# kdsuneraavinash/CH-Bin

Measured on AMD Instinct MI355X. Metric: convex-hull QP distances/sec (+ end-to-end bin-assign wall-clock), N=100000 D=136 B=64, higher is better.
Workload: dtype f64

## Files before the change

### ch-bin_amd/csrc/aux_kernels.hip

```cpp
#include "chb_internal.h"

namespace chb {
thread_local Gate g_gate;
namespace {

__global__ void fill_i32_kernel(int *p, int v, int n, Gate gate)
{
    CHB_GATE(gate);
    const int i = blockIdx.x * blockDim.x + threadIdx.x;
    if (i < n) p[i] = v;
}

__global__ void batch_close_kernel(int *labels, int *inb, const int *bq, const int *lab, int K)
{
    const int i = blockIdx.x * blockDim.x + threadIdx.x;
    if (i < K) {
        const int p = bq[i];
        labels[p] = lab[i];
        inb[p] = -1;
    }
}


__device__ __forceinline__ int member_key(int l, int p, const float4 *ms, const float *shell_inv, int nsh)
// ... 246 lines not shown
            const int e = atomicAdd(&cnt[rb[t]], 1);
            memb_id[e] = bq[i];
            memb_code[e] = -(i + 1);
        }
    }
    for (int i = tid + 1024 * kReg; i < K; i += 1024) {
        const int a = lab_prev[i];
        if (a >= 0 && a < B) {
            const int e = atomicAdd(&cnt[a], 1);
            memb_id[e] = bq[i];
            memb_code[e] = lab_old ? (i + 1) : (-(1 << 30) - i);
        }
        if (lab_old) {
            const int b = lab_old[i];
            if (b >= 0 && b < B) {
                const int e = atomicAdd(&cnt[b], 1);
                memb_id[e] = bq[i];
                memb_code[e] = -(i + 1);
            }
        }
    }
}

__global__ __launch_bounds__(256) void argmin_kernel(const double *dist, const int *lab_old, int *lab_prev,
                              int pos_begin, int pos_end, int B, int *lab_new, double *mind, double *second,
                              int *first_change, int in_place, Gate gate)
{
    CHB_GATE(gate);
    const int j = threadIdx.x & 7;
    const int pos = pos_begin + (int)((blockIdx.x * blockDim.x + threadIdx.x) >> 3);
    const bool valid = pos < pos_end;
    double best = kInf, runner = kInf;
    int bc = -1;
    if (valid) {
        const double *row = dist + (size_t)pos * B;
        for (int c = j; c < B; c += 8) {
            const double d = row[c];
            if (best > d) { runner = best; best = d; bc = c; }
            else if (runner > d) runner = d;
        }
    }
#pragma unroll
    for (int off = 1; off < 8; off <<= 1) {
        const double ob = __shfl_xor(best, off, 64), orr = __shfl_xor(runner, off, 64);
        const int oc = __shfl_xor(bc, off, 64);
        const bool take = ob < best || (ob == best && oc >= 0 && (bc < 0 || oc < bc));
// ... 363 lines not shown
}
void launch_batch_close(int *labels, int *inb, const int *bq, const int *lab, int K, hipStream_t s)
{
    if (K > 0) hipLaunchKernelGGL(batch_close_kernel, dim3((K + 255) / 256), dim3(256), 0, s, labels, inb, bq, lab, K);
}

void launch_bucket_base(const int *labels, int *inb, int N, int B, int *cnt, int *bin_ptr,
                        int *cursor, int *memb_id, int *pad_ptr, int *zero_me, hipStream_t s, const int *open_bq,
                        int open_K, int *open_lab_old, const SegPlan *seg, int *stats, const void *ms,
                        const float *shell_inv, int nsh)
{
    if (ms == nullptr || shell_inv == nullptr || nsh < 1) nsh = 1;
    const float4 *ms4 = reinterpret_cast<const float4 *>(ms);
    int blocks = (N + 255) / 256;
    if (blocks > 1024) blocks = 1024;
    hipLaunchKernelGGL(count_base_kernel, dim3(blocks), dim3(256), B * nsh * sizeof(int), s, labels, inb, N, B, cnt, open_bq,
                       open_K, open_lab_old, ms4, shell_inv, nsh, g_gate);
    hipLaunchKernelGGL(scan_kernel, dim3(1), dim3(256), 0, s, cnt, B, nsh, bin_ptr, cursor, pad_ptr, zero_me,
                       seg ? *seg : SegPlan{}, stats, g_gate);
    hipLaunchKernelGGL(fill_base_kernel, dim3((N + 255) / 256), dim3(256), 2 * B * nsh * sizeof(int), s, labels, inb, N, B,
                       cursor, memb_id, ms4, shell_inv, nsh, g_gate);
}

void launch_bucket_batch(const int *lab_prev, const int *lab_old, const int *bq, int K, int B,
                         int *cnt, int *bin_ptr, int *cursor, int *memb_id, int *memb_code, int *pad_ptr,
                         int *first_change, int *n_slow, int *nflag, hipStream_t s, void *bb_zero)
{
    (void)cnt; (void)cursor;
    hipLaunchKernelGGL(bucket_batch_kernel, dim3(1), dim3(1024), sizeof(int) * ((size_t)B + 2048), s, lab_prev,
                       lab_old, bq, K, B, bin_ptr, pad_ptr, memb_id, memb_code, first_change, n_slow, nflag,
                       reinterpret_cast<float4 *>(bb_zero), g_gate);
}

void launch_argmin(const double *dist, const int *lab_old, int *lab_prev, int pos_begin,
                   int pos_end, int B, int *lab_new, double *mind, double *second, int *first_change, bool in_place,
                   hipStream_t s)
{
    const int n = pos_end - pos_begin;
    if (n > 0)
        hipLaunchKernelGGL(argmin_kernel, dim3((n + 31) / 32), dim3(256), 0, s, dist, lab_old, lab_prev, pos_begin, pos_end, B,
                           lab_new, mind, second, first_change, in_place ? 1 : 0, g_gate);
}

}
```

### ch-bin_amd/csrc/chb_api.hip

```cpp
#include "chb_internal.h"
#include "../../include/chbin_hip.h"

#include <dlfcn.h>
#include <rccl/rccl.h>

#include <algorithm>
#include <cmath>
#include <cstdio>
#include <cstring>
#include <map>
#include <string>
#include <unordered_set>
#include <vector>

using namespace chb;

namespace {

thread_local std::string g_err;

int fail(int code, const std::string &msg)
{
    g_err = msg;
    return code;
// ... 92 lines not shown
    size_t cap = 0;
    hipError_t ensure(size_t n)
    {
        if (n <= cap) return hipSuccess;
        if (p) (void)hipHostFree(p);
        p = nullptr; cap = 0;
        hipError_t e = hipHostMalloc((void **)&p, std::max<size_t>(n, 1) * sizeof(T), hipHostMallocDefault);
        if (e == hipSuccess) cap = n;
        return e;
    }
    void release() { if (p) (void)hipHostFree(p); p = nullptr; cap = 0; }
    PinBuf() = default;
    PinBuf(const PinBuf &) = delete;
    PinBuf &operator=(const PinBuf &) = delete;
    ~PinBuf() { release(); }
};

}

struct PackBufs {
    DevBuf<unsigned short> Z;
    DevBuf<float> bias, sn, cs, cb, bb, tsn;
    DevBuf<int> pad_ptr;
    hipError_t ensure(size_t rows, size_t B, size_t Dz)
    {
        hipError_t e;
        if ((e = Z.ensure((rows + 64) * Dz)) != hipSuccess) return e;
        DevBuf<float> *f[] = {&bias, &sn, &cs, &cb};
        for (auto *b : f)
            if ((e = b->ensure(rows + 64)) != hipSuccess) return e;
        if ((e = bb.ensure(4 * B)) != hipSuccess) return e;
        if ((e = tsn.ensure(rows / 32 + B + 68)) != hipSuccess) return e;
        return pad_ptr.ensure(B + 1);
    }
    void release()
    {
        Z.release(); bias.release(); sn.release(); cs.release(); cb.release();
        bb.release(); tsn.release(); pad_ptr.release();
    }
    chb::MemberPack view()
    {
        return chb::MemberPack{Z.p, bias.p, sn.p, cs.p, cb.p, tsn.p, pad_ptr.p, reinterpret_cast<float4 *>(bb.p)};
    }
};

struct Switches {
    bool use_prefilter = true;
    bool allow_fused = true;
    bool fused_ptr64 = false;
    bool speculate = true;
    bool force_gather = false;
    bool allow_segments = true;
    bool fused_stripe = true;
    bool pp_allowed = true;
    bool pool_allowed = true, pool_force = false;
    bool allow_skip = true;
};

struct chb_ctx {
    int dev = 0;
    Switches sw;
// ... 99 lines not shown
    hipStream_t rc_copy = nullptr;
    hipEvent_t rc_up[2] = {nullptr, nullptr}, rc_done[2] = {nullptr, nullptr}, rc_down[2] = {nullptr, nullptr};
    DevBuf<int> xq, xhull, xcnt;
    DevBuf<double> xdist, xalpha, xpts;
    int prof = 0;
    std::map<std::string, ProfEntry> prof_acc;
    std::vector<Pending> pending;
    int64_t stats[4] = {0, 0, 0, 0};
    int64_t stats_seg_batches = 0;
    int64_t stats_lookahead = 0;
    int64_t stats_lookahead_failed = 0;
    ncclComm_t comm = nullptr;
    int rank = 0, world = 1;
    chb_allgather_fn hook = nullptr;
    void *hook_user = nullptr;
    std::vector<char> hook_send, hook_recv;
    double hint_base_members = 0.0, hint_batch_entries = 0.0;
#ifdef CHB_DEV_KNOBS
    struct DevKnobs {
        bool sl_bounds = false, sl_validate = false;
        int inject_short = 0, sl_bpw = 0, skip_never = 0;
        std::string sl_dbg;
        int64_t pack_rebuild_at = -1;
        bool hook_spec = false, local_verdict = false, skip_stats_on = false;
        int skip_stats[3] = {0, 0, 0};
        int batches = 0, launches = 0;
        DevBuf<int> viol, verr;
        DevBuf<unsigned long long> dbg;
    } dk;
#endif

    Lists L0() { return Lists{l0d.p, l0i.p, l0c.p}; }
    Lists L1() { return Lists{l1d.p, l1i.p, l1c.p}; }
    Lists L2() { return Lists{l2d.p, l2i.p, l2c.p}; }
    Lists Lcur() { return (round_in_batch & 1) ? L2() : L1(); }
    Lists Lprev() { return (round_in_batch & 1) ? L1() : L2(); }

    TopmArgs topm_args(int lo, int hi)
    {
        TopmArgs a{};
        a.X = X.p; a.Dp = Dp; a.bq = bq_cur; a.pos_begin = lo; a.pos_end = hi; a.B = B; a.m = m; a.Kcap = Kcap;
        return a;
    }
    ShortlistArgs shortlist_args(int lo, int hi)
    {
        ShortlistArgs a{};
// ... 111 lines not shown
    HIPCHK(h->bin_ptr.ensure(B + 1));
    HIPCHK(h->cursor.ensure(B * (size_t)kShells));
    HIPCHK(h->memb_id.ensure((size_t)h->N));
    HIPCHK(h->cnt2.ensure(B));
    HIPCHK(h->bin_ptr2.ensure(B + 1));
    HIPCHK(h->cursor2.ensure(B));
    HIPCHK(h->memb2_id.ensure(2 * K));
    HIPCHK(h->memb2_code.ensure(2 * K));
    if (h->pf_fit) {
        HIPCHK(h->cand.ensure(K * B * (size_t)kCandCap));
        HIPCHK(h->cand_cnt.ensure(K * B));
        HIPCHK(h->active.ensure(K * B));
        HIPCHK(h->n_active.ensure(1));
        HIPCHK(h->act_blk.ensure((K * B + 4095) / 4096 + 1));
        HIPCHK(h->flags64.ensure(B * ((K + kQTile - 1) / kQTile)));
        HIPCHK(h->flaglist.ensure(B * ((K + kQTile - 1) / kQTile)));
        HIPCHK(h->nflag.ensure(1));
        HIPCHK(h->flaglist2.ensure(B * ((K + kQTile - 1) / kQTile)));
        HIPCHK(h->nflag2.ensure(1));
        launch_fill_i32(h->flags64.p, 0, (int)(B * ((K + kQTile - 1) / kQTile)), h->stream);
        HIPCHK(h->overflow.ensure(1));
        HIPCHK(h->pk.ensure((size_t)h->N + 32 * B, B, (size_t)h->Dz));
        HIPCHK(h->pk2.ensure(2 * K + 32 * B, B, (size_t)h->Dz));
        h->seg_gcap = (int)std::min<size_t>(64, B / 4 + 1);
        HIPCHK(h->qord.ensure(K));
        HIPCHK(h->home.ensure(B));
        HIPCHK(h->seg_nseg.ensure(1));
        HIPCHK(h->seg_gflag.ensure(B));
        HIPCHK(h->seg_items.ensure(16 * (size_t)h->seg_gcap));
        if (h->fused) {
            for (int i = 0; i < 2; ++i) {
                HIPCHK(h->candu[i].ensure(K * B * (size_t)kCandCapU));
                HIPCHK(h->candu_cnt[i].ensure(K * B));
            }
            HIPCHK(h->slow.ensure(K * B));
            HIPCHK(h->n_slow.ensure(1));
            { const size_t had = h->short_cnt.cap; HIPCHK(h->short_cnt.ensure(1)); if (!had) HIPCHK(hipMemsetAsync(h->short_cnt.p, 0, sizeof(int), h->stream)); }
            HIPCHK(h->tau.ensure(K * B));
        }
    }
    h->Kcap = Kcap;
    return CHB_OK;
}

int fit_begin_impl(chb_ctx *h, int64_t B, const int64_t *initial, int m, bool sync = true)
{
// ... 138 lines not shown
void read_switches(chb_ctx *h)
{
    auto flag = [](const char *name, bool &v) { if (const char *e = getenv(name)) v = atoi(e) != 0; };
    Switches &w = h->sw;
    flag("CHB_PREFILTER", w.use_prefilter);
    flag("CHB_FUSED", w.allow_fused);
    flag("CHB_FUSED_PTR64", w.fused_ptr64);
    flag("CHB_SPECULATE", w.speculate);
    flag("CHB_FORCE_GATHER", w.force_gather);
    flag("CHB_SEGMENTS", w.allow_segments);
    flag("CHB_FUSED_STRIPE", w.fused_stripe);
    flag("CHB_PACK_INCR", w.pp_allowed);
    flag("CHB_TILE_SKIP", w.allow_skip);
    if (const char *e = getenv("CHB_POOL_TAU")) { w.pool_allowed = atoi(e) != 0; w.pool_force = atoi(e) == 2; }
#ifdef CHB_DEV_KNOBS
    auto &d = h->dk;
    d.sl_bounds = getenv("CHB_SL_BOUNDS") != nullptr;
    d.sl_validate = getenv("CHB_SL_VALIDATE") != nullptr;
    if (const char *e = getenv("CHB_SL_INJECT_SHORT")) d.inject_short = atoi(e);
    if (const char *e = getenv("CHB_SL_BPW")) d.sl_bpw = atoi(e);
    if (const char *e = getenv("CHB_SKIP_NEVER")) d.skip_never = atoi(e);
    if (const char *e = getenv("CHB_SL_DBG")) d.sl_dbg = e;
    if (const char *e = getenv("CHB_PACK_REBUILD_AT")) d.pack_rebuild_at = atoll(e);
    flag("CHB_DEV_HOOK_SPEC", d.hook_spec);
    flag("CHB_DEV_LOCAL_VERDICT", d.local_verdict);
    if (const char *e = getenv("CHB_DEV_SKIP_STATS"))
        d.skip_stats_on = sscanf(e, "%d,%d,%d", &d.skip_stats[0], &d.skip_stats[1], &d.skip_stats[2]) == 3;
#endif
}

#ifdef CHB_DEV_KNOBS
constexpr size_t kDbgWords = (size_t)65536 * 16;
int sl_bpw(const chb_ctx *h) { return h->dk.sl_bpw; }

int dev_shortlist_args(chb_ctx *h, ShortlistArgs &pa, bool skip_on, bool pp_now)
{
    auto &d = h->dk;
    if (skip_on && d.skip_never) pa.skip = 1 | 2 * d.skip_never;
    if (!d.sl_dbg.empty() && ++d.launches == 10) {
        HIPCHK(d.dbg.ensure(kDbgWords));
        HIPCHK(hipMemsetAsync(d.dbg.p, 0, kDbgWords * 8, h->stream));
        pa.dbg = d.dbg.p;
    }
    if (d.sl_bounds) {
        HIPCHK(d.viol.ensure(8));
        HIPCHK(hipMemsetAsync(d.viol.p, 0, 8 * sizeof(int), h->stream));
// ... 157 lines not shown
            RescoreArgs ra = h->rescore_args(q_lo, q_hi);
            ra.out = h->L0();
            Timed t(h, "rescore", (double)(q_hi - q_lo) * h->B);
            launch_rescore(ra, s);
        } else {
            a.out = Lists{nullptr, nullptr, nullptr};
            a.cand_out = h->cand.p; a.cand_cnt_out = h->cand_cnt.p; a.cand_cap = kCandCap;
            a.tau_out = h->tau.p; a.S = h->shadow_scale;
        }
        {
            Timed t(h, "topm_fallback", 0.0);
            launch_topm_flagged(a, h->flags64.p, fb_list, fb_n, s);
        }
        if (fusedp && !pp_now) { const int r_ = dev_shortlist_check(h, skip_on, qord_p); if (r_) return r_; }
    } else {
        Timed t(h, "topm_base", (double)(q_hi - q_lo) * h->hint_base_members);
        if (h->m > kMaxM) launch_topm_generic(a, s); else launch_topm(a, s);
    }
    HIPCHK(hipGetLastError());
    h->batch_open = true;
    return CHB_OK;
}

ShortlistArgs batch_entry_shortlist(chb_ctx *h, int lo, int hi)
{
    launch_pack_centered(h->X.p, h->D, h->Dp, h->memb2_id.p, h->memb2_code.p, h->bin_ptr2.p, h->B, 2 * h->K,
                         h->centers.p, h->mu_g.p, h->shadow_scale, h->Dz, h->pk2.view(), h->stream);
    ShortlistArgs pa = h->shortlist_args(lo, hi);
    pa.P = h->pk2.view(); pa.bin_ptr = h->bin_ptr2.p; pa.memb_id = h->memb2_id.p; pa.update = true;
    return pa;
}

void round_fused(chb_ctx *h, int lo, int hi, TopmArgs a)
{
    hipStream_t s = h->stream;
    const int cur = h->round_in_batch & 1;
    ShortlistArgs pa = batch_entry_shortlist(h, lo, hi);
    pa.tau_in = h->tau.p; pa.cand = h->candu[cur].p; pa.cand_cnt = h->candu_cnt[cur].p; pa.cand_cap = kCandCapU;
    {
        Timed t(h, "prefilter_update", (double)(hi - lo) * h->hint_batch_entries);
        launch_shortlist(pa, h->flags64.p, sl_bpw(h), s);
    }
    {
        a.in = a.out = Lists{nullptr, nullptr, nullptr};
        a.cand_out = h->candu[cur].p; a.cand_cnt_out = h->candu_cnt[cur].p; a.cand_cap = kCandCapU;
        Timed t(h, "topm_fallback", 0.0);
        launch_topm_flagged(a, h->flags64.p, h->flaglist.p, h->nflag.p, s);
    }
    FusedArgs f = h->fused_args(lo, hi);
    f.cand = h->cand.p; f.cand_cnt = h->cand_cnt.p; f.candu = h->candu[cur].p; f.candu_cnt = h->candu_cnt[cur].p;
    if (h->round_in_batch > 0) { f.candp = h->candu[cur ^ 1].p; f.candp_cnt = h->candu_cnt[cur ^ 1].p; }
    f.slow = h->slow.p; f.n_slow = h->n_slow.p; f.bin_ptr = h->bin_ptr.p; f.short_cnt = h->short_cnt.p;
// ... 38 lines not shown
        Timed t(h, "topm_fallback", 0.0);
        launch_topm_flagged(a, h->flags64.p, h->flaglist.p, h->nflag.p, s);
    }
    return CHB_OK;
}

void round_lists_plain(chb_ctx *h, int lo, int hi, const TopmArgs &a)
{
    Timed t(h, "topm_update", (double)(hi - lo) * h->hint_batch_entries);
    if (h->m > kMaxM) launch_topm_generic(a, h->stream); else launch_topm(a, h->stream);
}

int batch_round_dev(chb_ctx *h, int active)
{
    hipStream_t s = h->stream;
    const int lo = std::max(active, h->q_lo), hi = h->q_hi;
    if (hi <= lo) launch_fill_i32(h->fc_cur + kSlotFirstChange, h->K, 1, s);
    const bool fusedp = h->fused && h->lists_valid == false;
    if (hi > lo) {
        {
            Timed t(h, "bucket", (double)h->K);
            launch_bucket_batch(h->lab_prev.p, h->lab_old.p, h->bq_cur, h->K, h->B, h->cnt2.p, h->bin_ptr2.p, h->cursor2.p,
                                h->memb2_id.p, h->memb2_code.p, h->pk2.pad_ptr.p, h->fc_cur + kSlotFirstChange,
                                fusedp ? h->n_slow.p : nullptr, h->nflag.p, s, (h->pf_fit && h->pk2.bb.p) ? h->pk2.bb.p : nullptr);
        }
        TopmArgs a = h->topm_args(lo, hi);
        a.bin_ptr = h->bin_ptr2.p; a.memb_id = h->memb2_id.p; a.memb_code = h->memb2_code.p;
        a.in = h->L0(); a.out = h->Lcur();
        if (fusedp) round_fused(h, lo, hi, a);
        else {
            if (h->pf_fit && h->cand.p) { const int r_ = round_lists_shortlist(h, lo, hi, a); if (r_) return r_; }
            else round_lists_plain(h, lo, hi, a);
            QpArgs q = h->qp_args(lo, hi);
            q.lists = h->Lcur();
            q.prev = h->round_in_batch > 0 ? h->Lprev() : Lists{nullptr, nullptr, nullptr};
            Timed t(h, "hull_qp", (double)(hi - lo) * h->B);
            if (h->m > kMaxM) launch_hull_generic(q, s); else launch_hull_qp(q, s);
        }
        {
            Timed t(h, "argmin", (double)(hi - lo));
            launch_argmin(h->dist.p, h->lab_old.p, h->lab_prev.p, lo, hi, h->B, h->lab_new.p, h->mind.p,
                          h->want_margin ? h->mind2.p : nullptr, h->fc_cur + kSlotFirstChange, h->argmin_in_place, s);
        }
        h->stats[2] += (int64_t)(hi - lo) * h->B;
    }
    HIPCHK(hipGetLastError());
    h->stats[1] += 1;
// ... 1520 lines not shown
```

### ch-bin_amd/csrc/chb_internal.h

```cpp
#pragma once
#include <hip/hip_runtime.h>
#include <stdint.h>

#include <vector>

namespace chb {

struct Gate {
    const int *flag = nullptr;
    int need = 0;
};
extern thread_local Gate g_gate;
#define CHB_GATE(g) do { if ((g).flag != nullptr && *(g).flag < (g).need) return; } while (0)

constexpr double kInf = __builtin_huge_val();
constexpr int kMaxM = 16;
constexpr int kMaxMGeneric = 64;
constexpr int kQTile = 64;
constexpr int kPTile = 64;
constexpr int kKChunk = 8;
constexpr int kLdsStride = 66;

struct Lists {
    double *d;
// ... 11 lines not shown
    const int *bin_cnt = nullptr;
    const int *memb_code;
    int B, m, Kcap;
    Lists in;
    Lists out;
    int *cand_out = nullptr, *cand_cnt_out = nullptr;
    int cand_cap = 0;
    float *tau_out = nullptr;
    double S = 1.0;
};

void launch_topm(const TopmArgs &a, hipStream_t s);
void launch_topm_generic(const TopmArgs &a, hipStream_t s);
void launch_topm_flagged(const TopmArgs &a, int *flags64, const int *flaglist, const int *nflag, hipStream_t s);

constexpr int kCandCap = 128;
constexpr int kCandCapU = 32;

struct MemberPack {
    unsigned short *Z;
    float *bias;
    float *sn;
    float *cs, *cb;
    float *tsn;
    int *pad_ptr;
    float4 *bb;
    const int *nt = nullptr;
};
int shortlist_list_len(int m);
int shadow_row_elems(int D);
void launch_global_center(const double *X, int N, int D, int Dp, double *part, int part_blocks, double *mu_g,
                          unsigned int *rmax, hipStream_t s);
void launch_global_shadow(const double *X, int N, int D, int Dp, const double *mu_g, double S,
                          unsigned short *Gs, int Dz, void *gq, hipStream_t s);
void launch_bin_centers(const double *X, int D, int Dp, const int *memb_id, const int *bin_ptr, int B,
                        double *centers, hipStream_t s);
void launch_shell_scale(const void *ms, const int *memb_id, const int *bin_ptr, int B, int nsh, float *shell_inv,
                        hipStream_t s);
void launch_sample_shadow(const double *X, int D, int Dp, const int *ids, int n, int *labels,
                          int B, const double *centers, const double *mu_g, double S, unsigned short *Zs,
                          int Dz, void *ms, const int *new_lab, int *inb, hipStream_t s);
void launch_pack_centered(const double *X, int D, int Dp, const int *memb_id, const int *memb_code,
                          const int *bin_ptr, int B, int rows_hint, const double *centers, const double *mu_g,
                          double S, int Dz, const MemberPack &P, hipStream_t s);
void launch_pack_build(const unsigned short *Zs, const void *ms, int D, int Dz, const int *memb_id, const int *bin_ptr,
                       int B, int rows_hint, const MemberPack &P, bool shells, hipStream_t s);
void launch_query_norms(const double *X, int D, int Dp, int N, int B, const double *centers, double S, void *qn,
// ... 177 lines not shown
};
constexpr int kRecruitChunk = 16384;
constexpr int kRecruitMaxBins = 8192;
void launch_recruit(const RecruitArgs &a, hipStream_t s);
void launch_recruit_reduce(const double *dist, int nq, int B, int *bin, double *mind, double *margin, hipStream_t s);

void launch_fill_i32(int *p, int v, int n, hipStream_t s);
void launch_copy_i32(int *dst, const int *src, int n, hipStream_t s);
#ifdef CHB_DEV_KNOBS
void launch_validate_batch(const int *cand, const int *cand_cnt, int B, int Kcap, int pos_begin, int pos_end, int cap, int N,
                           const int *bin_ptr, const int *memb_id, const int *qord, int m, int *err, hipStream_t s);
void launch_inject_short(int *cand_cnt, int B, int Kcap, int pos, const int *bin_ptr, int m, hipStream_t s);
#endif
void launch_batch_close(int *labels, int *inb, const int *bq, const int *lab, int K, hipStream_t s);
void launch_bucket_base(const int *labels, int *inb, int N, int B, int *cnt, int *bin_ptr,
                        int *cursor, int *memb_id, int *pad_ptr, int *zero_me, hipStream_t s,
                        const int *open_bq = nullptr, int open_K = 0, int *open_lab_old = nullptr,
                        const SegPlan *seg = nullptr, int *stats = nullptr, const void *ms = nullptr,
                        const float *shell_inv = nullptr, int nsh = 1);
constexpr int kShells = 32;
constexpr int kMaxKeys = 8192;
void launch_bucket_batch(const int *lab_prev, const int *lab_old, const int *bq, int K, int B,
                         int *cnt, int *bin_ptr, int *cursor, int *memb_id, int *memb_code, int *pad_ptr,
                         int *first_change, int *n_slow, int *nflag, hipStream_t s, void *bb_zero = nullptr);
void launch_first_change(const int *lab_new, const int *lab_prev, int p0, int K, int *first_change,
                         hipStream_t s);
void launch_guess(const double *list_d, const int *list_cnt, const int *lab_old, int p0, int p1,
                  int B, int m, int Kcap, int *lab_prev, hipStream_t s);
void launch_guess_near(const float *tau, const int *lab_old, int p0, int p1, int B, int Kcap, int *lab_prev,
                       hipStream_t s);
enum SlotWord {
    kSlotFirstChange = 0,
    kSlotMaxTiles = 1,
    kSlotTotalTiles = 2,
    kSlotSkipped = 3,
    kSlotSeen = 4,
    kSlotUnloaded = 5,
    kSlotMark = 6,
    kSlotPoolCand = 7,
    kSlotPoolPairs = 8,
    kSlotHome = 9,
    kSlotShortCnt = 12,
    kSlotPackErr = 13,
};
constexpr int kSlotInts = 16;
enum FrameWord {
    kFrameTag = 0,
// ... 30 lines not shown
```

### ch-bin_amd/csrc/prefilter_kernels.hip

```cpp
#include "chb_internal.h"

#include <float.h>
#include <math.h>
#include <stdlib.h>

#include <algorithm>

namespace chb {
namespace {

using f16x8 = __attribute__((ext_vector_type(8))) _Float16;
using f32x16 = __attribute__((ext_vector_type(16))) float;
using f32x4 = __attribute__((ext_vector_type(4))) float;

constexpr int kBiasCols = 3;
constexpr int kBiasExp = 14;
constexpr float kGamma = 2.5e-5f;
constexpr float kSlack = 1e-6f;
constexpr int kPfW = 4;
constexpr int kPfQ = 32 * kPfW;
constexpr int kPfP = 32;
constexpr int kWideMaxSlices = 4;

__device__ __forceinline__ float round_up_f32(double v)
{
    float f = (float)v;
    if ((double)f < v) f = nextafterf(f, INFINITY);
    return f;
}

__device__ __forceinline__ unsigned short f16_shadow(double zs, double &back)
{
    float f = (float)zs;
    f = fminf(fmaxf(f, -65504.f), 65504.f);
    const _Float16 hv = (_Float16)f;
    back = (double)(float)hv;
    return __builtin_bit_cast(unsigned short, hv);
}

__device__ __forceinline__ void bound_max(float *slot, float v)
{
    if (v == v && v > 0.f) atomicMax(reinterpret_cast<unsigned int *>(slot), __float_as_uint(v));
}
// ... 975 lines not shown

template <int ML>
__device__ __forceinline__ void list_insert_desc(float (&l)[ML], float v)
{
#pragma unroll
    for (int i = 0; i < ML; ++i) {
        const float hi = fmaxf(l[i], v);
        v = fminf(l[i], v);
        l[i] = hi;
    }
}

__device__ __noinline__ void shortlist_flush_call(const unsigned *pool, int npark, int *cnt, const int *qpos, int *cand_bin,
                                                  int cand_cap, const int *memb, int lane)
{
    for (int i = lane; i < npark; i += 64) {
        const unsigned en = pool[i];
        const int qc = (int)(en >> 27), e = (int)(en & ((1u << 27) - 1u));
        const int off = atomicAdd(&cnt[qc], 1);
        if (off < cand_cap) cand_bin[(size_t)qpos[qc] * cand_cap + off] = memb[e];
    }
}

template <int ML, bool UPD, int KS, int SEG = 0, bool SKIP = false, bool POOL = false, bool WORK = false>
__global__ __launch_bounds__(64 * kPfW, (ML <= 5 && (KS == 9 || (!UPD && SEG != 2))) ? 4 : 3) void shortlist_kernel(ShortlistArgs a, int nqt, int nchunk,
                                                                         int bpw, int *flags64, int nqt64, Gate gate)
{
    CHB_GATE(gate);
    static_assert(!WORK || (!UPD && SEG == 0 && !SKIP && !POOL), "the work-list form is the plain base build");
    static_assert(SEG == 0 || !UPD, "segments exist for base members only");
    static_assert(!POOL || (!UPD && SEG == 0), "threshold pools serve the ordinary base launch");
#ifdef CHB_DEV_KNOBS
    const unsigned long long dbg_t0 = wall_clock64();
    int dbg_tiles = 0;
#endif
    constexpr int CPR = 2 * KS;
    constexpr int ROWB = 32 * KS;
    constexpr int TILEB = kPfP * ROWB;
    constexpr int METAB = 512;
    constexpr bool kFour = sl_four(KS, UPD, ML, SEG);
    constexpr int BUFB = kFour ? TILEB : TILEB + METAB;
    constexpr int NBUF = 3;
    constexpr int kPoolW = shortlist_pool_entries(ML);
    extern __shared__ __attribute__((aligned(16))) unsigned char smem[];
    unsigned *sPool = reinterpret_cast<unsigned *>(smem + NBUF * BUFB);
    int *sCnt = reinterpret_cast<int *>(sPool + kPfW * kPoolW);
// ... 93 lines not shown
        const int pch = (w + kPfW * j) * 64 + lane;
        const int r = pch / CPR, cs = pch - r * CPR;
        const int f = KS == 9 ? ((r >> 4) & 1) : ((r >> 2) & 3);
        src_off[j] = (r * CPR + (cs ^ f)) * 16;
    }
    int n_w = 0;
#pragma unroll
    for (int j = 0; j < 3; ++j) n_w += (w + kPfW * j < KS) ? 1 : 0;
    n_w += (UPD && w == 3) ? 1 : 0;
    n_w += (UPD && w == 2) ? 1 : 0;
    const unsigned char *zall = reinterpret_cast<const unsigned char *>(a.P.Z);

    int ic = c0, it = 0, isw = (UPD || SEG == 2) ? 1 : 0, ibuf = 0;
    int irow0 = 0, int_ = 0;
    bool ivalid = false;
    const long long pool_delta = (long long)reinterpret_cast<unsigned long long>(a.pool.Z) -
                                 (long long)reinterpret_cast<unsigned long long>(a.P.Z);
    long long ioff = 0;
    int brow0 = 0, bnt = 0;
#define CHB_SL_ISSUE_SEEK()                                                                        \
    {                                                                                              \
        ivalid = false;                                                                            \
        while (ic < c1) {                                                                          \
            irow0 = a.P.pad_ptr[ic];                                                               \
            int_ = a.P.nt != nullptr ? a.P.nt[ic] : (a.P.pad_ptr[ic + 1] - irow0) / kPfP;          \
            if (SEG == 0 && !UPD && a.seg.gflag != nullptr && a.seg.gflag[ic] >= 0) int_ = 0;     \
            if (SEG != 0) { irow0 += seg_tb * kPfP; int_ = min(int_, seg_te) - seg_tb; }           \
            if (int_ > 0) { ivalid = true; break; }                                                \
            ++ic;                                                                                  \
        }                                                                                          \
        if (POOL && ivalid) {                                                                      \
            brow0 = irow0; bnt = int_;                                                             \
            const bool pm_ = pool_mode_of(ic);                                                     \
            ioff = pm_ ? pool_delta + (long long)((ic * a.B + h_lo) * kPoolRows) * ROWB : (long long)irow0 * ROWB; \
            int_ = pm_ ? n_home : int_;                                                            \
        }                                                                                          \
    }
#ifdef CHB_DEV_KNOBS
#define CHB_SL_BOUNDS_DMA()                                                                        \
        if (a.viol != nullptr) {                                                                   \
            const long long bo_ = POOL ? ioff + (long long)it * kPfP * ROWB : (long long)row_ * ROWB; \
            const bool in_pack_ = bo_ >= 0 && bo_ + (long long)kPfP * ROWB <= a.viol_rows * ROWB;  \
            const bool in_pool_ = POOL && bo_ >= pool_delta && bo_ + (long long)kPfP * ROWB <= pool_delta + a.viol_pool_rows * ROWB; \
            if (!in_pack_ && !in_pool_) {                                                          \
                if (tid == 0 && atomicCAS(&a.viol[0], 0, 1) == 0) {                                \
                    a.viol[1] = ic; a.viol[2] = it; a.viol[3] = (int)(bo_ / ROWB); a.viol[4] = isw; a.viol[5] = int_; a.viol[6] = (int)(pool_delta >> 8); a.viol[7] = (int)blockIdx.x; \
                }                                                                                  \
                src_ = zall;                                                                       \
// ... 38 lines not shown
    int fbase0, fbase1;
    if (KS == 9) {
        const int f = (col >> 4) & 1;
        fbase0 = col * ROWB + ((h ^ f) << 4);
        fbase1 = fbase0 + 32;
    } else {
        const int f0 = (col >> 2) & 1, f1 = (col >> 3) & 1;
        fbase0 = col * ROWB + (f1 << 5) + ((h ^ f0) << 4);
        fbase1 = col * ROWB + ((1 ^ f1) << 5) + ((h ^ f0) << 4);
    }
    const unsigned ent0 = ((unsigned)col << 27) | (unsigned)(4 * h);

#ifdef CHB_DEV_KNOBS
#define CHB_SL_BOUNDS_FLUSH()                                                                      \
            if (a.viol != nullptr && ((long long)mb_ + e >= a.viol_members || e < 0)) {            \
                if (atomicCAS(&a.viol[0], 0, 2) == 0) { a.viol[1] = c; a.viol[2] = e; a.viol[3] = mb_; a.viol[4] = qc; a.viol[7] = (int)blockIdx.x; } \
                continue;                                                                          \
            }
#else
#define CHB_SL_BOUNDS_FLUSH()
#endif
#define CHB_SL_FLUSH()                                                                             \
    {                                                                                              \
        const int mb_ = a.bin_ptr[c];                                                              \
        const int npark_ = wcnt < kPoolW ? wcnt : kPoolW;                                          \
        if (SEG == 2) {                                                                            \
            for (int i = lane; i < npark_; i += 64)                                                \
                atomicAdd(&sCnt[32 * w + (int)(sPool[w * kPoolW + i] >> 27)], 1);                  \
            __builtin_amdgcn_fence(__ATOMIC_ACQ_REL, "wavefront");                                 \
            if (h == 0) {                                                                          \
                const int nq_ = sCnt[32 * w + col];                                                \
                int gb_ = 0;                                                                       \
                if (nq_ > 0 && qvalid) gb_ = atomicAdd(&a.cand_cnt[slot], nq_);                    \
                seg_over = seg_over || gb_ + nq_ > a.cand_cap;                                     \
                sGb[32 * w + col] = gb_;                                                           \
                sCnt[32 * w + col] = 0;                                                            \
            }                                                                                      \
            __builtin_amdgcn_fence(__ATOMIC_ACQ_REL, "wavefront");                                 \
        }                                                                                          \
        for (int i = lane; i < npark_; i += 64) {                                                  \
            const unsigned en = sPool[w * kPoolW + i];                                             \
            const int qc = (int)(en >> 27), e = (int)(en & ((1u << 27) - 1u));                     \
            int off = atomicAdd(&sCnt[32 * w + qc], 1);                                            \
            if (SEG == 2) off += sGb[32 * w + qc];                                                 \
            CHB_SL_BOUNDS_FLUSH()                                                                  \
            if (off < a.cand_cap)                                                                  \
                a.cand[(kSeated ? (size_t)c * a.Kcap + sQpos[32 * w + qc] : (size_t)c * a.Kcap + pos0 + 32 * w + qc) * a.cand_cap + off] = a.memb_id[mb_ + e]; \
        }                                                                                          \
        if (SEG == 2) {                                                                            \
            __builtin_amdgcn_fence(__ATOMIC_ACQ_REL, "wavefront");                                 \
            if (h == 0) sCnt[32 * w + col] = 0;                                                    \
        }                                                                                          \
    }
    int cbuf = 0;
    int wt_seen = 0, wt_skipped = 0, wt_unloaded = 0;
    int pool_cand = 0, pool_pairs = 0;
    for (int c = c0; c < c1; ++c) {
        const int row0 = a.P.pad_ptr[c];
        int ntile = a.P.nt != nullptr ? a.P.nt[c] : (a.P.pad_ptr[c + 1] - row0) / kPfP;
        if (SEG == 0 && !UPD && a.seg.gflag != nullptr && a.seg.gflag[c] >= 0) continue;
        if (SEG != 0) ntile = min(ntile, seg_te) - seg_tb;
        bool seg_over = false;
        const size_t slot = (size_t)c * a.Kcap + (qvalid ? qpos : a.pos_end - 1);
        float4 bb = a.P.bb[c];
        if (UPD) bb.y = sqrtf(bb.y) * (1.0f + 1e-6f);
        const float2 qn2 = a.qn[(size_t)sidx * a.B + c];
        const float E = ((UPD ? 1.2e-7f * bb.z : 2.0f * bb.w) + a.gamma * (1.001f * bb.z + 2.0f * snq * bb.y)) *
                        (1.0f + 4.0f * kSlack);
        const float rgq = rg * (1.0f + 4.0f * kSlack);
        const float *tsn_c = UPD ? nullptr : a.P.tsn + (row0 >> 5) + seg_tb;

        const float nj_hi = (qn2.x + E) * (1.0f + kSlack);
        const float nj_lo = (qn2.y - E) * (qn2.y > E ? (1.0f - kSlack) : (1.0f + kSlack));
        const float rsum = bb.x * (1.0f + kSlack);
        const float zn_lo = sqrtf(fmaxf(nj_lo, 0.f)) * (1.0f - 4.0f * kSlack) - rsum;
        float tau_run = INFINITY, hi_s1 = INFINITY;
#ifdef CHB_DEV_KNOBS
        const bool kSkipNever = (a.skip & 2) != 0;
        const bool kNoExit = (a.skip & 4) != 0, kNoWaveSkip = (a.skip & 8) != 0, kNoMidFlush = (a.skip & 16) != 0;
#else
        constexpr bool kSkipNever = false;
#endif
        constexpr bool can_skip = SKIP;
        float lb[ML];
// ... 380 lines not shown
#pragma unroll
    for (int j = 0; j < 3; ++j) {
        const int pch = (w + kPfW * j) * 64 + lane;
        const int r = pch / CPR, cs = pch - r * CPR;
        const int f = (r >> 4) & 1;
        src_off[j] = r * ROWB + (cs ^ f) * 16;
    }
    int n_w = 0;
#pragma unroll
    for (int j = 0; j < 3; ++j) n_w += (w + kPfW * j < KS) ? 1 : 0;
    n_w += (UPD && w == 3) ? 1 : 0;
    n_w += (UPD && w == 2) ? 1 : 0;
    const unsigned char *zall = reinterpret_cast<const unsigned char *>(a.P.Z);

    int ic = c0, it = 0, is = 0, isw = UPD ? 1 : 0, ibuf = 0;
    int irow0 = 0, int_ = 0;
    bool ivalid = false;
    int n_issued = 0, n_consumed = 0;
    auto issue_seek = [&]() __attribute__((always_inline)) {
        ivalid = false;
        while (ic < c1) {
            irow0 = a.P.pad_ptr[ic];
            int_ = a.P.nt != nullptr ? a.P.nt[ic] : (a.P.pad_ptr[ic + 1] - irow0) / kPfP;
            if (int_ > 0) { ivalid = true; break; }
            ++ic;
        }
    };
    auto issue = [&]() __attribute__((always_inline)) {
        unsigned char *dst_ = smem + ibuf * BUFB;
        const size_t row_ = (size_t)irow0 + (size_t)it * kPfP;
        const unsigned char *src_ = zall + row_ * ROWB + is * SLB;
#pragma unroll
        for (int j = 0; j < 3; ++j)
            if (w + kPfW * j < KS)
                __builtin_amdgcn_global_load_lds(src_ + src_off[j],
                    (__attribute__((address_space(3))) void *)(dst_ + (w + kPfW * j) * 1024), 16, 0, 0);
        if (UPD && w == 3) {
            const float *p_ = (h ? a.P.cs : a.P.bias) + row_ + col;
            __builtin_amdgcn_global_load_lds(p_, (__attribute__((address_space(3))) void *)(dst_ + TILEB), 4, 0, 0);
        }
        if (UPD && w == 2) {
            const float *p_ = (h ? a.P.sn : a.P.cb) + row_ + col;
            __builtin_amdgcn_global_load_lds(p_, (__attribute__((address_space(3))) void *)(dst_ + TILEB + 256), 4, 0, 0);
        }
        if (++ibuf == NBUF) ibuf = 0;
        ++n_issued;
        if (++is == NS) {
            is = 0;
            if (++it == int_) {
                it = 0;
                if (!UPD && isw == 0) isw = 1;
                else { isw = UPD ? 1 : 0; ++ic; issue_seek(); }
            }
        }
    };
    issue_seek();
    if (ivalid) issue();
    if (ivalid) issue();

    const int fbase0 = col * SLB + ((h ^ ((col >> 4) & 1)) << 4);
    const unsigned ent0 = ((unsigned)col << 27) | (unsigned)(4 * h);

    int cbuf = 0;
    for (int c = c0; c < c1; ++c) {
        const int row0 = a.P.pad_ptr[c];
        const int ntile = a.P.nt != nullptr ? a.P.nt[c] : (a.P.pad_ptr[c + 1] - row0) / kPfP;
        const size_t slot = (size_t)c * a.Kcap + (qvalid ? qpos : a.pos_end - 1);
        float4 bb = a.P.bb[c];
        if (UPD) bb.y = sqrtf(bb.y) * (1.0f + 1e-6f);
        const float2 qn2 = a.qn[(size_t)sidx * a.B + c];
        const float E = ((UPD ? 1.2e-7f * bb.z : 2.0f * bb.w) + a.gamma * (1.001f * bb.z + 2.0f * snq * bb.y)) *
                        (1.0f + 4.0f * kSlack);
        const float rgq = rg * (1.0f + 4.0f * kSlack);
        const float *tsn_c = UPD ? nullptr : a.P.tsn + (row0 >> 5);
        const float nj_hi = (qn2.x + E) * (1.0f + kSlack);
        const float nj_lo = (qn2.y - E) * (qn2.y > E ? (1.0f - kSlack) : (1.0f + kSlack));
        const float rsum = bb.x * (1.0f + kSlack);
        float lb[ML];
#pragma unroll
        for (int i = 0; i < ML; ++i) lb[i] = i < ML - m ? INFINITY : -INFINITY;
        float thr_s = -INFINITY;
        float thr2 = qvalid ? -FLT_MAX : INFINITY;
        if (UPD && qvalid) {
            float tau = INFINITY;
            if (a.tau_in != nullptr) tau = a.tau_in[slot];
            else if (a.seed.cnt[slot] >= m) tau = round_up_f32(a.seed.d[slot * m + m - 1] * a.S) * (1.0f + kSlack);
            if (tau < INFINITY) {
                const float hi = tau * (1.0f + 4.0f * kSlack) + rsum;
                thr2 = -0.5f * (hi * hi * (1.0f + 4.0f * kSlack) - nj_lo);
            }
        }
        if (h == 0) sCnt[32 * w + col] = 0;
        const bool tile_best = ntile >= a.tile_best_min && 4 * ntile >= m * m && !(!UPD && a.skip != 0);
        const int kmax = (ML > 8 && !tile_best && ntile >= a.tile_best_min && !(!UPD && a.skip != 0)) ? a.tile_k2 : 0x7fffffff;
        int wcnt = 0;
        auto flush = [&]() __attribute__((always_inline)) {
            const int mb_ = a.bin_ptr[c];
            const int npark_ = wcnt < kPoolW ? wcnt : kPoolW;
            for (int i = lane; i < npark_; i += 64) {
                const unsigned en = sPool[w * kPoolW + i];
                const int qc = (int)(en >> 27), e = (int)(en & ((1u << 27) - 1u));
                const int off = atomicAdd(&sCnt[32 * w + qc], 1);
                if (off < a.cand_cap)
                    a.cand[((size_t)c * a.Kcap + pos0 + 32 * w + qc) * a.cand_cap + off] = a.memb_id[mb_ + e];
            }
        };

        for (int sweep = UPD ? 1 : 0; sweep < 2; ++sweep) {
            const float rgs = (sweep ? rg : -rg) * (1.0f + kSlack);
            if (!UPD && sweep == 1) {
                float mg[ML];
#pragma unroll
                for (int i = 0; i < ML; ++i) mg[i] = lb[i];
#pragma unroll
                for (int i = 0; i < ML; ++i) {
                    const float o = __shfl_xor(lb[i], 32, 64);
                    list_insert_desc<ML>(mg, i >= ML - m ? o : -INFINITY);
                }
                const float ms = mg[ML - 1];
                float tau = INFINITY;
// ... 437 lines not shown
```

Measured before the change: 647.4 million.

## Order batch-entry buckets by query position and restrict shortlist scans to per-tile windows

```diff
diff --git a/ch-bin_amd/csrc/aux_kernels.hip b/ch-bin_amd/csrc/aux_kernels.hip
--- a/ch-bin_amd/csrc/aux_kernels.hip
+++ b/ch-bin_amd/csrc/aux_kernels.hip
@@ -292,6 +292,141 @@
     }
 }
 
+__device__ __forceinline__ int scan_parts_wave(int *part, int lane)
+{
+    int loc = 0;
+    for (int i = 0; i < 16; ++i) loc += part[16 * lane + i];
+    int inc = loc;
+#pragma unroll
+    for (int off = 1; off < 64; off <<= 1) {
+        const int o = __shfl_up(inc, off, 64);
+        if (lane >= off) inc += o;
+    }
+    int run = inc - loc;
+    for (int i = 0; i < 16; ++i) {
+        const int v = part[16 * lane + i];
+        part[16 * lane + i] = run;
+        run += v;
+    }
+    return run;
+}
+
+__global__ __launch_bounds__(1024) void bucket_batch_ordered_kernel(const int *lab_prev, const int *lab_old, const int *bq,
+                                                                    int K, int B, int nch, int shift, int q_lo,
+                                                                    int q_hi, int *bin_ptr, int *pad_ptr, int *memb_id,
+                                                                    int *memb_code, int4 *twin,
+                                                                    int *first_change, int *n_slow, int *nflag,
+                                                                    float4 *bb_zero, Gate gate)
+{
+    CHB_GATE(gate);
+    extern __shared__ int sh[];
+    const int ncell = 2 * B * nch;
+    int *cnt = sh, *part = sh + ncell + 1;
+    const int tid = threadIdx.x;
+    if (bb_zero != nullptr)
+        for (int b = tid; b < B; b += 1024) bb_zero[b] = make_float4(0.f, 0.f, 0.f, 0.f);
+    if (tid == 0) {
+        if (first_change) *first_change = K;
+        if (n_slow) *n_slow = 0;
+        if (nflag) *nflag = 0;
+    }
+    for (int c = tid; c < ncell; c += 1024) cnt[c] = 0;
+    __syncthreads();
+    auto cell_of = [&](int l, int run, int i) { return (l >= 0 && l < B) ? (2 * l + run) * nch + (i >> shift) : -1; };
+    constexpr int kReg = 8;
+    int ra[kReg], rb[kReg];
+#pragma unroll
+    for (int t = 0; t < kReg; ++t) {
+        const int i = tid + 1024 * t;
+        ra[t] = i < K ? cell_of(lab_prev[i], 1, i) : -1;
+        rb[t] = i < K ? cell_of(lab_old[i], 0, i) : -1;
+    }
+#pragma unroll
+    for (int t = 0; t < kReg; ++t) {
+        if (ra[t] >= 0) atomicAdd(&cnt[ra[t]], 1);
+        if (rb[t] >= 0) atomicAdd(&cnt[rb[t]], 1);
+    }
+    for (int i = tid + 1024 * kReg; i < K; i += 1024) {
+        const int a = cell_of(lab_prev[i], 1, i), b = cell_of(lab_old[i], 0, i);
+        if (a >= 0) atomicAdd(&cnt[a], 1);
+        if (b >= 0) atomicAdd(&cnt[b], 1);
+    }
+    __syncthreads();
+    {
+        const int per = (ncell + 1023) / 1024;
+        const int c0 = min(ncell, tid * per), c1 = min(ncell, c0 + per);
+        int s = 0;
+        for (int c = c0; c < c1; ++c) s += cnt[c];
+        part[tid] = s;
+        __syncthreads();
+        if (tid < 64) {
+            const int total = scan_parts_wave(part, tid);
+            if (tid == 63) { cnt[ncell] = total; bin_ptr[B] = total; }
+        }
+        __syncthreads();
+        int run = part[tid];
+        for (int c = c0; c < c1; ++c) { const int v = cnt[c]; cnt[c] = run; run += v; }
+        __syncthreads();
+    }
+    {
+        const int per = (B + 1023) / 1024;
+        const int b0 = min(B, tid * per), b1 = min(B, b0 + per);
+        int sp = 0;
+        for (int b = b0; b < b1; ++b) sp += (cnt[(2 * b + 2) * nch] - cnt[2 * b * nch] + 31) / 32 * 32;
+        part[tid] = sp;
+        __syncthreads();
+        if (tid < 64) {
+            const int ptotal = scan_parts_wave(part, tid);
+            if (tid == 63) pad_ptr[B] = ptotal;
+        }
+        __syncthreads();
+        int prun = part[tid];
+        for (int b = b0; b < b1; ++b) {
+            bin_ptr[b] = cnt[2 * b * nch];
+            pad_ptr[b] = prun;
+            prun += (cnt[(2 * b + 2) * nch] - cnt[2 * b * nch] + 31) / 32 * 32;
+        }
+    }
+    __syncthreads();
+    const int nqt = (q_hi - q_lo + kSlQTile - 1) / kSlQTile;
+    for (int x = tid; x < B * nqt; x += 1024) {
+        const int b = x / nqt, t = x - b * nqt;
+        const int p0 = q_lo + t * kSlQTile, p1 = min(p0 + kSlQTile, q_hi) - 1;
+        const int e0 = cnt[2 * b * nch];
+        const int tb = (cnt[2 * b * nch + (p0 >> shift)] - e0) >> 5;
+        const int te = (cnt[(2 * b + 1) * nch + (p1 >> shift) + 1] - e0 + 31) >> 5;
+        twin[x] = make_int4(pad_ptr[b] + 32 * tb, te - tb, e0 + 32 * tb, 0);
+    }
+    __syncthreads();
+#pragma unroll
+    for (int t = 0; t < kReg; ++t) {
+        const int i = tid + 1024 * t;
+        if (ra[t] >= 0) {
+            const int e = atomicAdd(&cnt[ra[t]], 1);
+            memb_id[e] = bq[i];
+            memb_code[e] = i + 1;
+        }
+        if (rb[t] >= 0) {
+            const int e = atomicAdd(&cnt[rb[t]], 1);
+            memb_id[e] = bq[i];
+            memb_code[e] = -(i + 1);
+        }
+    }
+    for (int i = tid + 1024 * kReg; i < K; i += 1024) {
+        const int a = cell_of(lab_prev[i], 1, i), b = cell_of(lab_old[i], 0, i);
+        if (a >= 0) {
+            const int e = atomicAdd(&cnt[a], 1);
+            memb_id[e] = bq[i];
+            memb_code[e] = i + 1;
+        }
+        if (b >= 0) {
+            const int e = atomicAdd(&cnt[b], 1);
+            memb_id[e] = bq[i];
+            memb_code[e] = -(i + 1);
+        }
+    }
+}
+
 __global__ __launch_bounds__(256) void argmin_kernel(const double *dist, const int *lab_old, int *lab_prev,
                               int pos_begin, int pos_end, int B, int *lab_new, double *mind, double *second,
                               int *first_change, int in_place, Gate gate)
@@ -701,11 +836,31 @@
                        cursor, memb_id, ms4, shell_inv, nsh, g_gate);
 }
 
+int batch_window_shift(int K, int B, int cells)
+{
+    if (K <= 0 || B <= 0) return 0;
+    for (int shift = 7; shift < 31; ++shift) {
+        const long long nch = ((K - 1) >> shift) + 1;
+        if (2LL * B * nch <= cells) return shift;
+        if (nch == 1) break;
+    }
+    return 0;
+}
+
 void launch_bucket_batch(const int *lab_prev, const int *lab_old, const int *bq, int K, int B,
                          int *cnt, int *bin_ptr, int *cursor, int *memb_id, int *memb_code, int *pad_ptr,
-                         int *first_change, int *n_slow, int *nflag, hipStream_t s, void *bb_zero)
+                         int *first_change, int *n_slow, int *nflag, hipStream_t s, void *bb_zero, int *twin, int twin_shift,
+                         int q_lo, int q_hi)
 {
     (void)cnt; (void)cursor;
+    if (twin != nullptr && K > 0 && q_lo >= 0 && q_lo < q_hi && q_hi <= K) {
+        const int nch = ((K - 1) >> twin_shift) + 1;
+        hipLaunchKernelGGL(bucket_batch_ordered_kernel, dim3(1), dim3(1024), sizeof(int) * (2 * (size_t)B * nch + 1 + 1024), s,
+                           lab_prev, lab_old, bq, K, B, nch, twin_shift, q_lo, q_hi, bin_ptr, pad_ptr, memb_id, memb_code,
+                           reinterpret_cast<int4 *>(twin), first_change, n_slow, nflag, reinterpret_cast<float4 *>(bb_zero),
+                           g_gate);
+        return;
+    }
     hipLaunchKernelGGL(bucket_batch_kernel, dim3(1), dim3(1024), sizeof(int) * ((size_t)B + 2048), s, lab_prev,
                        lab_old, bq, K, B, bin_ptr, pad_ptr, memb_id, memb_code, first_change, n_slow, nflag,
                        reinterpret_cast<float4 *>(bb_zero), g_gate);
diff --git a/ch-bin_amd/csrc/chb_api.hip b/ch-bin_amd/csrc/chb_api.hip
--- a/ch-bin_amd/csrc/chb_api.hip
+++ b/ch-bin_amd/csrc/chb_api.hip
@@ -138,6 +138,8 @@
     DevBuf<unsigned short> Z;
     DevBuf<float> bias, sn, cs, cb, bb, tsn;
     DevBuf<int> pad_ptr;
+    DevBuf<int> twin;
+    hipError_t ensure_windows(size_t B, size_t K) { return twin.ensure(4 * B * ((K + kSlQTile - 1) / kSlQTile + 1)); }
     hipError_t ensure(size_t rows, size_t B, size_t Dz)
     {
         hipError_t e;
@@ -152,7 +154,7 @@
     void release()
     {
         Z.release(); bias.release(); sn.release(); cs.release(); cb.release();
-        bb.release(); tsn.release(); pad_ptr.release();
+        bb.release(); tsn.release(); pad_ptr.release(); twin.release();
     }
     chb::MemberPack view()
     {
@@ -298,6 +300,7 @@
         int inject_short = 0, sl_bpw = 0, skip_never = 0;
         std::string sl_dbg;
         int64_t pack_rebuild_at = -1;
+        int batch_cells = -1;
         bool hook_spec = false, local_verdict = false, skip_stats_on = false;
         int skip_stats[3] = {0, 0, 0};
         int batches = 0, launches = 0;
@@ -455,6 +458,7 @@
         HIPCHK(h->overflow.ensure(1));
         HIPCHK(h->pk.ensure((size_t)h->N + 32 * B, B, (size_t)h->Dz));
         HIPCHK(h->pk2.ensure(2 * K + 32 * B, B, (size_t)h->Dz));
+        HIPCHK(h->pk2.ensure_windows(B, K));
         h->seg_gcap = (int)std::min<size_t>(64, B / 4 + 1);
         HIPCHK(h->qord.ensure(K));
         HIPCHK(h->home.ensure(B));
@@ -639,6 +643,7 @@
     if (const char *e = getenv("CHB_SKIP_NEVER")) d.skip_never = atoi(e);
     if (const char *e = getenv("CHB_SL_DBG")) d.sl_dbg = e;
     if (const char *e = getenv("CHB_PACK_REBUILD_AT")) d.pack_rebuild_at = atoll(e);
+    if (const char *e = getenv("CHB_BATCH_CELLS")) d.batch_cells = std::max(0, std::min(atoi(e), kBatchCells));
     flag("CHB_DEV_HOOK_SPEC", d.hook_spec);
     flag("CHB_DEV_LOCAL_VERDICT", d.local_verdict);
     if (const char *e = getenv("CHB_DEV_SKIP_STATS"))
@@ -842,12 +847,22 @@
     return CHB_OK;
 }
 
+int entry_window_shift(const chb_ctx *h, int lo, int hi)
+{
+    if (!h->pf_fit || h->pk2.twin.p == nullptr || lo < 0 || lo >= hi || hi > h->K) return 0;
+#ifdef CHB_DEV_KNOBS
+    if (h->dk.batch_cells >= 0) return batch_window_shift(h->K, h->B, h->dk.batch_cells);
+#endif
+    return batch_window_shift(h->K, h->B);
+}
+
 ShortlistArgs batch_entry_shortlist(chb_ctx *h, int lo, int hi)
 {
     launch_pack_centered(h->X.p, h->D, h->Dp, h->memb2_id.p, h->memb2_code.p, h->bin_ptr2.p, h->B, 2 * h->K,
                          h->centers.p, h->mu_g.p, h->shadow_scale, h->Dz, h->pk2.view(), h->stream);
     ShortlistArgs pa = h->shortlist_args(lo, hi);
     pa.P = h->pk2.view(); pa.bin_ptr = h->bin_ptr2.p; pa.memb_id = h->memb2_id.p; pa.update = true;
+    pa.P.twin = entry_window_shift(h, lo, hi) ? reinterpret_cast<const int4 *>(h->pk2.twin.p) : nullptr;
     return pa;
 }
 
@@ -932,7 +947,8 @@
             Timed t(h, "bucket", (double)h->K);
             launch_bucket_batch(h->lab_prev.p, h->lab_old.p, h->bq_cur, h->K, h->B, h->cnt2.p, h->bin_ptr2.p, h->cursor2.p,
                                 h->memb2_id.p, h->memb2_code.p, h->pk2.pad_ptr.p, h->fc_cur + kSlotFirstChange,
-                                fusedp ? h->n_slow.p : nullptr, h->nflag.p, s, (h->pf_fit && h->pk2.bb.p) ? h->pk2.bb.p : nullptr);
+                                fusedp ? h->n_slow.p : nullptr, h->nflag.p, s, (h->pf_fit && h->pk2.bb.p) ? h->pk2.bb.p : nullptr,
+                                entry_window_shift(h, lo, hi) ? h->pk2.twin.p : nullptr, entry_window_shift(h, lo, hi), lo, hi);
         }
         TopmArgs a = h->topm_args(lo, hi);
         a.bin_ptr = h->bin_ptr2.p; a.memb_id = h->memb2_id.p; a.memb_code = h->memb2_code.p;
diff --git a/ch-bin_amd/csrc/chb_internal.h b/ch-bin_amd/csrc/chb_internal.h
--- a/ch-bin_amd/csrc/chb_internal.h
+++ b/ch-bin_amd/csrc/chb_internal.h
@@ -57,7 +57,10 @@
     float *bias;
     float *sn;
     float *cs, *cb;
-    float *tsn;
+    union {
+        float *tsn;
+        const int4 *twin;
+    };
     int *pad_ptr;
     float4 *bb;
     const int *nt = nullptr;
@@ -281,7 +284,11 @@
 constexpr int kMaxKeys = 8192;
 void launch_bucket_batch(const int *lab_prev, const int *lab_old, const int *bq, int K, int B,
                          int *cnt, int *bin_ptr, int *cursor, int *memb_id, int *memb_code, int *pad_ptr,
-                         int *first_change, int *n_slow, int *nflag, hipStream_t s, void *bb_zero = nullptr);
+                         int *first_change, int *n_slow, int *nflag, hipStream_t s, void *bb_zero = nullptr,
+                         int *twin = nullptr, int twin_shift = 0, int q_lo = 0, int q_hi = 0);
+constexpr int kSlQTile = 128;
+constexpr int kBatchCells = 14336;
+int batch_window_shift(int K, int B, int cells = kBatchCells);
 void launch_first_change(const int *lab_new, const int *lab_prev, int p0, int K, int *first_change,
                          hipStream_t s);
 void launch_guess(const double *list_d, const int *list_cnt, const int *lab_old, int p0, int p1,
diff --git a/ch-bin_amd/csrc/prefilter_kernels.hip b/ch-bin_amd/csrc/prefilter_kernels.hip
--- a/ch-bin_amd/csrc/prefilter_kernels.hip
+++ b/ch-bin_amd/csrc/prefilter_kernels.hip
@@ -19,6 +19,7 @@
 constexpr float kSlack = 1e-6f;
 constexpr int kPfW = 4;
 constexpr int kPfQ = 32 * kPfW;
+static_assert(kPfQ == kSlQTile, "the batch-entry tile windows are per query tile of the shortlist kernels");
 constexpr int kPfP = 32;
 constexpr int kWideMaxSlices = 4;
 
@@ -1040,6 +1041,8 @@
     }
 }
 
+__device__ __forceinline__ int4 entry_window(const MemberPack &P, int c, int nqt, int qt) { return P.twin[c * nqt + qt]; }
+
 template <int ML, bool UPD, int KS, int SEG = 0, bool SKIP = false, bool POOL = false, bool WORK = false>
 __global__ __launch_bounds__(64 * kPfW, (ML <= 5 && (KS == 9 || (!UPD && SEG != 2))) ? 4 : 3) void shortlist_kernel(ShortlistArgs a, int nqt, int nchunk,
                                                                          int bpw, int *flags64, int nqt64, Gate gate)
@@ -1179,8 +1182,13 @@
     {                                                                                              \
         ivalid = false;                                                                            \
         while (ic < c1) {                                                                          \
+            if (UPD && a.P.twin != nullptr) {                                                      \
+                const int4 win_ = entry_window(a.P, ic, nqt, qt);                                  \
+                irow0 = win_.x; int_ = win_.y;                                                     \
+            } else {                                                                               \
             irow0 = a.P.pad_ptr[ic];                                                               \
             int_ = a.P.nt != nullptr ? a.P.nt[ic] : (a.P.pad_ptr[ic + 1] - irow0) / kPfP;          \
+            }                                                                                      \
             if (SEG == 0 && !UPD && a.seg.gflag != nullptr && a.seg.gflag[ic] >= 0) int_ = 0;     \
             if (SEG != 0) { irow0 += seg_tb * kPfP; int_ = min(int_, seg_te) - seg_tb; }           \
             if (int_ > 0) { ivalid = true; break; }                                                \
@@ -1265,7 +1273,7 @@
 #endif
 #define CHB_SL_FLUSH()                                                                             \
     {                                                                                              \
-        const int mb_ = a.bin_ptr[c];                                                              \
+        const int mb_ = (UPD && a.P.twin != nullptr) ? entry_window(a.P, c, nqt, qt).z : a.bin_ptr[c]; \
         const int npark_ = wcnt < kPoolW ? wcnt : kPoolW;                                          \
         if (SEG == 2) {                                                                            \
             for (int i = lane; i < npark_; i += 64)                                                \
@@ -1303,6 +1311,7 @@
         int ntile = a.P.nt != nullptr ? a.P.nt[c] : (a.P.pad_ptr[c + 1] - row0) / kPfP;
         if (SEG == 0 && !UPD && a.seg.gflag != nullptr && a.seg.gflag[c] >= 0) continue;
         if (SEG != 0) ntile = min(ntile, seg_te) - seg_tb;
+        if (UPD && a.P.twin != nullptr) ntile = entry_window(a.P, c, nqt, qt).y;
         bool seg_over = false;
         const size_t slot = (size_t)c * a.Kcap + (qvalid ? qpos : a.pos_end - 1);
         float4 bb = a.P.bb[c];
@@ -1729,6 +1738,10 @@
         while (ic < c1) {
             irow0 = a.P.pad_ptr[ic];
             int_ = a.P.nt != nullptr ? a.P.nt[ic] : (a.P.pad_ptr[ic + 1] - irow0) / kPfP;
+            if (UPD && a.P.twin != nullptr) {
+                const int4 win = entry_window(a.P, ic, nqt, qt);
+                irow0 = win.x; int_ = win.y;
+            }
             if (int_ > 0) { ivalid = true; break; }
             ++ic;
         }
@@ -1771,7 +1784,8 @@
     int cbuf = 0;
     for (int c = c0; c < c1; ++c) {
         const int row0 = a.P.pad_ptr[c];
-        const int ntile = a.P.nt != nullptr ? a.P.nt[c] : (a.P.pad_ptr[c + 1] - row0) / kPfP;
+        int ntile = a.P.nt != nullptr ? a.P.nt[c] : (a.P.pad_ptr[c + 1] - row0) / kPfP;
+        if (UPD && a.P.twin != nullptr) ntile = entry_window(a.P, c, nqt, qt).y;
         const size_t slot = (size_t)c * a.Kcap + (qvalid ? qpos : a.pos_end - 1);
         float4 bb = a.P.bb[c];
         if (UPD) bb.y = sqrtf(bb.y) * (1.0f + 1e-6f);
@@ -1802,7 +1816,7 @@
         const int kmax = (ML > 8 && !tile_best && ntile >= a.tile_best_min && !(!UPD && a.skip != 0)) ? a.tile_k2 : 0x7fffffff;
         int wcnt = 0;
         auto flush = [&]() __attribute__((always_inline)) {
-            const int mb_ = a.bin_ptr[c];
+            const int mb_ = (UPD && a.P.twin != nullptr) ? entry_window(a.P, c, nqt, qt).z : a.bin_ptr[c];
             const int npark_ = wcnt < kPoolW ? wcnt : kPoolW;
             for (int i = lane; i < npark_; i += 64) {
                 const unsigned en = sPool[w * kPoolW + i];
```

Result: slower. 634.1 million (-2.1%).
